# SmallVCM/SmallVCM

Hardware: AMD Instinct MI355X
Metric: Mpaths/sec (light+camera), VCM scene 1 at 2048^2 (higher is better)
Workload: dtype f32; 1 GPU; scene 1 -a vcm 2048x2048 maxPathLength 10 minPathLength 0 radiusFactor 0.003 radiusAlpha 0.75 seed 1234, iterations 5..408 timed; parallelism=1 renderer(s) (iteration-parallel, smallvcm.cxx:61-108) on one GPU, 1 in flight

## Files before the change

### smallvcm_amd/csrc/vcm_api.hip

```cpp
#include <hip/hip_runtime.h>
#include <stdio.h>
#include <stdlib.h>
#include <string.h>
#include <string>
#include <new>
#include <mutex>
#include <vector>
#include <condition_variable>
#include <atomic>

#include "vcm_kernels.h"
#include "vcm_kat.h"
#include "scene_host.h"
#include "scene_kind.h"
#include "vcm_denoise.h"
#include "vcm_variance.h"
#include "vcm_robust.h"
#include "vcm_parts.h"

using namespace vcm;

static thread_local std::string g_err;
static thread_local bool g_hipFailed;
static int fail(const char *what, const char *detail)
// ... 78 lines not shown
#endif
struct vcm_ctx : Scratch {
    SceneHost *scene;
    bool useVM, useVC, lightTraceOnly, ppm;
    int renderer;
    float baseRadius, radiusAlpha;
    int seed, device, rank, world;
    int resX, resY, N, p0, nLocal;
    int iterations;

    hipStream_t stream;
    bool ownStream;
    hipStream_t side;
    hipEvent_t evFork, evBbox, evGrid;
    bool gridInFlight;
    hipStream_t splat;
    hipEvent_t evSplatFork, evSplatDone;
    hipEvent_t evSortFork, evSorted;
    hipEvent_t evZero;
    bool prezeroed, sortInFlight;
    bool splatInFlight;
    bool resolveInFlight;
    hipEvent_t evMergeDone, evSplatWork, evResolved;
    hipEvent_t evPreMerge;
    bool mergeInFlight;
    bool deviceReady;
    ArenaPool *pool;
    Arena *arena; bool holdsArena;

    DScene *dScene;
    char *dSceneBlob;
    float *dFb;
    unsigned char *dRngLight, *dRngCam;
    GridHeader *dHdr;
    unsigned long long *dStats;
    unsigned long long *dStatsRing;
    unsigned long long *dStamps;
    float radiusRing[VCM_STAMP_RING];
    double stampKHz;

    bool importedRecords;
    bool importedSorted;
    bool sortedExchange;
    SortedSlabs sortedIn;
    SpaceSlabs space; bool spaceSet, mergeImported;
    float presetMin[3];
    int *dSpaceMatrix, *dSpaceScanned, *dSpaceTotals, *dSpaceHist;
    int *dWhereDest, *dWherePos; size_t whereCap;
    F4 *fQ, *fRes; int *fKey, *fArrival, *fSorted, *fCount; size_t fCap;
    bool gridBuilt, cameraTraced, merged, splatsPending, recordsValid, countedInCamera, scatteredInDI, bboxPreset;
    bool bboxFromLight;
    bool bboxFinal;
    bool strictOrder;
    int mergeKind;
    int lastMergeKernel;
    SceneKind kind;
    bool envMap;
    bool lens;
    bool filter;
    bool pick;
    bool lights;
    bool intPhong;
    F4 *dGuide, *dAlbedo;
    F4 *dDnA, *dDnB, *dDenoised;
    bool featuresValid, denoisedValid;
    bool trackVariance;
    F4 *dVarPrev, *dVarMom;
    int robustBuckets, robustAlloc;
    F4 *dRobPrev, *dRobBuckets, *dRobOut;
    bool trackParts;
    float *dParts;
    F4 *dPartOut;
    int fbIterations;
    IterParams P;
    bool inIteration;
    hipEvent_t ev[EV_COUNT];
    bool evValid;
    unsigned long long *pend[2][4]; int nPend[2];
    vcm_stats lastStats;
};

template <unsigned Wrap, class F> static void launch_kind(const vcm_ctx *c, F &&f) { with_scene_kind<Wrap>(c->kind, SceneWrappers{ c->lens || c->filter, c->pick, c->lights }, f); }

typedef void (*MergeKernel)(const DScene *, IterParams, GridStore, VertexStore, const int *, const int *, unsigned long long *, int, StampArgs);
static MergeKernel merge_kernel(int mergeKind, bool intPhong)
{
    if (mergeKind == VCM_MERGE_PAIRS) return intPhong ? k_merge_pairs<true> : k_merge_pairs<false>;
    return intPhong ? k_merge_walk<true> : k_merge_walk<false>;
}

static int use_device(vcm_ctx *c) { HIPCHK(hipSetDevice(c->device)); return 0; }

static thread_local size_t g_allocBytes;
template <typename T> static int dalloc(T **p, size_t n)
{
    void *v = NULL;
    HIPCHK(hipMalloc(&v, (n ? n : 1) * sizeof(T)));
    g_allocBytes += (n ? n : 1) * sizeof(T);
    *p = (T *)v;
    return 0;
}
#define DFREE(p) do { if (p) { (void)hipFree(p); p = NULL; } } while (0)

static std::mutex g_arenaRegistryMutex;
static ArenaPool *g_pools[64];

// ... 463 lines not shown
    vcm_ctx *c = new (std::nothrow) vcm_ctx();
    if (!c) { delete h; fail("vcm_create", "out of host memory"); return NULL; }
    memset((void *)c, 0, sizeof(*c));
    c->scene = h;
    c->envMap = h->envW > 0;
    c->lens = h->lensRadius > 0.f;
    c->filter = h->filterKind != VCM_FILTER_BOX;
    c->pick = h->pickMode != VCM_LIGHT_PICK_UNIFORM;
    c->lights = c->pick && scene_host_has_new_lights(*h);
    scene_host_build_accel(*h, scene_host_force_bvh());
    switch (algorithm) {
    case VCM_ALGO_LIGHT_TRACE: c->lightTraceOnly = true; break;
    case VCM_ALGO_PPM: c->ppm = true; c->useVM = true; break;
    case VCM_ALGO_BPM: c->useVM = true; break;
    case VCM_ALGO_BPT: c->useVC = true; break;
    case VCM_ALGO_VCM: c->useVC = true; c->useVM = true; break;
    case VCM_ALGO_PATH_TRACE: c->renderer = 1; break;
    case VCM_ALGO_EYE_LIGHT: c->renderer = 2; break;
    default: delete h; delete c; fail("vcm_create", "unknown algorithm"); return NULL;
    }
    if (c->ppm) {
        for (const vcm_material &m : h->materials) {
            const bool hasNonSpecular = (vmax3(ld3(m.diffuse)) > 0) || (vmax3(ld3(m.phong)) > 0);
            const bool hasSpecular = (vmax3(ld3(m.mirror)) > 0) || (m.ior > 0);
            if (hasNonSpecular && hasSpecular) {
                fprintf(stderr, "smallvcm_amd: scene mixes specular and non-specular BSDFs in one material, "
                                "switching from PPM to BPM (vertexcm.hxx:262-275)\n");
                c->ppm = false;
                break;
            }
        }
    }
    c->baseRadius = radiusFactor * h->sceneRadius;
    c->radiusAlpha = radiusAlpha;
    c->seed = seed;
    c->device = device; c->rank = rank; c->world = worldSize;
    c->resX = (int)h->camera.resolution[0];
    c->resY = (int)h->camera.resolution[1];
    c->N = c->resX * c->resY;
    if (c->N <= 0) { delete h; delete c; fail("vcm_create", "empty resolution"); return NULL; }
    c->p0 = (int)((long long)c->N * rank / worldSize);
    c->nLocal = (int)((long long)c->N * (rank + 1) / worldSize) - c->p0;
    c->ownStream = true;
    if (worldSize == 1) {
        c->pool = pool_get(device);
        if (!c->pool) { delete h; delete c; fail("vcm_create", "device index out of range"); return NULL; }
        std::lock_guard<std::mutex> g(c->pool->m);
        c->pool->users++;
    } else {
        c->arena = arena_new(device, NULL);
    }
    const char *so = getenv("SMALLVCM_AMD_STRICT_ORDER");
    c->strictOrder = (so && so[0] == '1');
    { const char *e = getenv("SMALLVCM_AMD_SORTED_EXCHANGE");
      c->sortedExchange = worldSize > 1 && worldSize <= VCM_SORTED_MAX_SHARDS && c->useVM && !(e && e[0] == '0'); }
    { const char *e = getenv("SMALLVCM_AMD_MERGE");
      c->mergeKind = (e && !strcmp(e, "walk")) ? VCM_MERGE_WALK : (e && !strcmp(e, "pairs")) ? VCM_MERGE_PAIRS : VCM_MERGE_DEFAULT; }
    c->lastMergeKernel = 0;
    return c;
}

vcm_ctx *vcm_create_sharded(const vcm_scene_desc *scene, int algorithm, float radiusFactor, float radiusAlpha,
                            int seed, int device, int rank, int worldSize)
{
    if (!scene) { fail("vcm_create", "scene is NULL"); return NULL; }
    SceneHost *h = new (std::nothrow) SceneHost();
    std::string err;
    if (!h || !scene_host_from_desc(*scene, *h, err)) { delete h; fail("vcm_create", err.c_str()); return NULL; }
    return create_from_host(h, algorithm, radiusFactor, radiusAlpha, seed, device, rank, worldSize);
}

vcm_ctx *vcm_create_sharded2(const vcm_scene_desc2 *scene, int algorithm, float radiusFactor, float radiusAlpha,
                             int seed, int device, int rank, int worldSize)
{
    if (!scene) { fail("vcm_create2", "scene is NULL"); return NULL; }
    SceneHost *h = new (std::nothrow) SceneHost();
    std::string err;
    if (!h || !scene_host_from_desc2(*scene, *h, err)) { delete h; fail("vcm_create2", err.c_str()); return NULL; }
    return create_from_host(h, algorithm, radiusFactor, radiusAlpha, seed, device, rank, worldSize);
}

vcm_ctx *vcm_create_sharded3(const vcm_scene_desc3 *scene, int algorithm, float radiusFactor, float radiusAlpha,
                             int seed, int device, int rank, int worldSize)
{
    if (!scene) { fail("vcm_create3", "scene is NULL"); return NULL; }
    SceneHost *h = new (std::nothrow) SceneHost();
    std::string err;
    if (!h || !scene_host_from_desc3(*scene, *h, err)) { delete h; fail("vcm_create3", err.c_str()); return NULL; }
    return create_from_host(h, algorithm, radiusFactor, radiusAlpha, seed, device, rank, worldSize);
}

vcm_ctx *vcm_create_sharded4(const vcm_scene_desc4 *scene, int algorithm, float radiusFactor, float radiusAlpha,
                             int seed, int device, int rank, int worldSize)
{
    if (!scene) { fail("vcm_create4", "scene is NULL"); return NULL; }
    SceneHost *h = new (std::nothrow) SceneHost();
    std::string err;
    if (!h || !scene_host_from_desc4(*scene, *h, err)) { delete h; fail("vcm_create4", err.c_str()); return NULL; }
    return create_from_host(h, algorithm, radiusFactor, radiusAlpha, seed, device, rank, worldSize);
}

vcm_ctx *vcm_create_sharded5(const vcm_scene_desc5 *scene, int algorithm, float radiusFactor, float radiusAlpha,
                             int seed, int device, int rank, int worldSize)
{
    if (!scene) { fail("vcm_create5", "scene is NULL"); return NULL; }
    SceneHost *h = new (std::nothrow) SceneHost();
// ... 320 lines not shown
        hipLaunchKernelGGL(k_splat_apply, dim3(aux_blocks(c->nLocal)), dim3(256), 0, q, c->N, (const int *)pixStart,
                           (const F4 *)list, c->dFb, arrival, pixCount, splatLong);
        hipLaunchKernelGGL(k_splat_apply_long, dim3(1024), dim3(256), 0, q, (const int *)pixStart, (const F4 *)list,
                           c->dSplat, c->dFb, (const int *)arrival, (const int *)pixCount);
        HIPCHK(hipGetLastError());
        if (c->trackParts) {
            float *plane = c->dParts + (size_t)VCM_PART_LIGHT_TRACE * (size_t)c->N * 3;
            HIPCHK(hipMemsetAsync(pixCount, 0, sizeof(int), q));
            hipLaunchKernelGGL(k_splat_apply, dim3(aux_blocks(c->nLocal)), dim3(256), 0, q, c->N, (const int *)pixStart,
                               (const F4 *)list, plane, arrival, pixCount, splatLong);
            hipLaunchKernelGGL(k_splat_apply_long, dim3(1024), dim3(256), 0, q, (const int *)pixStart, (const F4 *)list,
                               c->dSplat, plane, (const int *)arrival, (const int *)pixCount);
            HIPCHK(hipGetLastError());
        }
        if (overlap) {
            HIPCHK(hipEventRecord(c->evSplatDone, q));
            c->splatInFlight = true;
        }
    }
    return 0;
}

static int vcm_trace_light_impl(vcm_ctx *c)
{
    if (!c || !c->inIteration) return fail("vcm_trace_light", "no iteration in progress");
    if (use_device(c)) return -1;
    if (c->renderer) {
        if (mark(c, EV_LIGHT_K0)) return -1;
        if (mark(c, EV_LIGHT_K1)) return -1;
        HIPCHK(hipMemsetAsync(c->dLocalTotal, 0, sizeof(int), c->stream));
        if (mark(c, EV_LIGHT)) return -1;
        hipLaunchKernelGGL(k_set_counts, dim3(1), dim3(1), 0, c->stream, c->dHdr, c->dLocalTotal, 1, 0, take_stamps(c, c->stream));
        HIPCHK(hipGetLastError());
        return 0;
    }
    int blocks, chunk;
    trace_launch_shape(c->nLocal, &blocks, &chunk, true);
    if (c->world == 1 && !c->strictOrder) {
        HIPCHK(hipEventRecord(c->evFork, c->stream));
        HIPCHK(hipStreamWaitEvent(c->side, c->evFork, 0));
        if (zero_ranges(c->side, c->useVM ? c->dQueryCount : NULL, c->useVM ? ((size_t)c->P.nBuckets + 1) * sizeof(int) : 0,
                        (c->useVM && !grid_sort_is_radix(c)) ? c->dCellCount : NULL, c->useVM ? ((size_t)c->P.nCells + 1) * sizeof(int) : 0,
                        (c->useVC || c->lightTraceOnly) ? c->dPixCount : NULL, ((size_t)c->N + 1) * sizeof(int))) return -1;
        HIPCHK(hipEventRecord(c->evZero, c->side));
        c->prezeroed = true;
    }
    if (mark(c, EV_LIGHT_K0)) return -1;
    const bool wf = !c->strictOrder;
    if (!wf && join_splats(c)) return -1;
    if (wf)
        launch_kind<kWrapPick>(c, [&](auto tag) {
            using S = typename decltype(tag)::type;
            hipLaunchKernelGGL((k_light_trace<1, S>), dim3(blocks), dim3(VCM_TRACE_BLOCK), 0, c->stream, c->dScene, c->P, c->store,
                               c->dFb, c->dRngLight, c->dStats, chunk, take_stamps(c, c->stream), c->vs.count + 16, c->dHdr);
        });
    else
        launch_kind<kWrapLens | kWrapPick>(c, [&](auto tag) {
            using S = typename decltype(tag)::type;
            hipLaunchKernelGGL((k_light_trace<0, S>), dim3(blocks), dim3(VCM_TRACE_BLOCK), 0, c->stream, c->dScene, c->P, c->store,
                               c->dFb, c->dRngLight, c->dStats, chunk, take_stamps(c, c->stream), c->vs.count + 16, c->dHdr);
        });
    HIPCHK(hipGetLastError());
    c->bboxFromLight = c->world == 1;
    if (mark(c, EV_LIGHT_K1)) return -1;
    if (launch_scan<unsigned char>(c, c->store.count, c->nLocal, c->dPathStart, c->dLocalTotal, 0)) return -1;
    if (c->mergeInFlight) { HIPCHK(hipStreamWaitEvent(c->stream, c->evMergeDone, 0)); c->mergeInFlight = false; }
    bool countsSet = false;
    if (c->useVM || wf) {
        c->recordsValid = c->useVM && c->world > 1 && !c->sortedExchange;
        const bool fold = c->world == 1;
        hipLaunchKernelGGL(k_compact_records, dim3(aux_blocks(c->nLocal)), dim3(256), 0, c->stream, (const DScene *)c->dScene, c->P, c->store, c->dPathStart,
                           c->dRecordsLocal, c->dSlotOfVertex, c->recordsValid ? 1 : 0, fold ? c->dHdr : (GridHeader *)NULL,
                           (const int *)c->dLocalTotal, (fold && c->bboxFromLight) ? 1 : 0);
        HIPCHK(hipGetLastError());
        countsSet = fold;
        if (fold && c->bboxFromLight) c->bboxFinal = true;
    }
    if (wf && (c->useVC || c->lightTraceOnly)) {
        c->splatsPending = true;
        if (c->world == 1 && flush_light_splats(c)) return -1;
    }
    if (mark(c, EV_LIGHT)) return -1;
    if (!countsSet) {
        hipLaunchKernelGGL(k_set_counts, dim3(1), dim3(1), 0, c->stream, c->dHdr, c->dLocalTotal, 1, 0, take_stamps(c, c->stream));
        HIPCHK(hipGetLastError());
    }
    return 0;
}

static int ensure_records(vcm_ctx *c)
{
    if (c->recordsValid || !c->useVM) return 0;
    hipLaunchKernelGGL(k_compact_records, dim3(aux_blocks(c->nLocal)), dim3(256), 0, c->stream, (const DScene *)c->dScene, c->P, c->store, c->dPathStart,
                       c->dRecordsLocal, c->dSlotOfVertex, 1, (GridHeader *)NULL, (const int *)c->dLocalTotal, 0);
    HIPCHK(hipGetLastError());
    c->recordsValid = true;
    return 0;
}

int vcm_light_records(vcm_ctx *c, void **devPtr, long long *count)
{
    if (scratch_readable(c, "vcm_light_records")) return -1;
    if (use_device(c)) return -1;
    int n = 0;
    if (devPtr && ensure_records(c)) return -1;
    HIPCHK(hipMemcpyAsync(&n, c->dLocalTotal, sizeof(int), hipMemcpyDeviceToHost, c->stream));
    HIPCHK(hipStreamSynchronize(c->stream));
    if (devPtr) *devPtr = c->dRecordsLocal;
    if (count) *count = n;
    return 0;
}

static int vcm_local_light_bbox_impl(vcm_ctx *c, float *min3, float *max3, long long *count)
// ... 282 lines not shown
    return 0;
}

static GridStore grid_of(vcm_ctx *c)
{
    GridStore grid;
    grid.cellStart = c->dCellStart; grid.gx = c->dGx; grid.gy = c->dGy; grid.gz = c->dGz; grid.gb = c->dGb; grid.g1 = c->dG1; grid.g2 = c->dG2; grid.g3 = c->dG3;
    grid.hdr = c->dHdr;
    return grid;
}

static int vcm_trace_camera_impl(vcm_ctx *c)
{
    if (!c || !c->inIteration) return fail("vcm_trace_camera", "no iteration in progress");
    if (use_device(c)) return -1;
    if (flush_light_splats(c)) return -1;
    c->cameraTraced = true;
    if (c->lightTraceOnly) return 0;
    int blocks, chunk;
    trace_launch_shape(c->nLocal, &blocks, &chunk);
    if (c->resolveInFlight) HIPCHK(hipStreamWaitEvent(c->stream, c->evResolved, 0));
    if (mark(c, EV_CAMERA_K0)) return -1;
    if (c->renderer) {
        if (c->renderer == 1)
            launch_kind<kWrapLens | kWrapPick>(c, [&](auto tag) {
                using S = typename decltype(tag)::type;
                hipLaunchKernelGGL((k_path_trace<S>), dim3(blocks), dim3(VCM_TRACE_BLOCK), 0, c->stream, c->dScene, c->P, c->dCamOut,
                                   c->dRngCam, c->dStats, chunk, take_stamps(c, c->stream), c->vs.count + 8);
            });
        else
            launch_kind<kWrapLens>(c, [&](auto tag) {
                using S = typename decltype(tag)::type;
                hipLaunchKernelGGL((k_eye_light<S>), dim3(2048), dim3(256), 0, c->stream, c->dScene, c->P, c->dCamOut, c->dRngCam,
                                   c->dStats, take_stamps(c, c->stream));
            });
        HIPCHK(hipGetLastError());
        if (mark(c, EV_CAMERA_K1)) return -1;
        if (mark(c, EV_CONNECT_K1)) return -1;
        return 0;
    }
    if (c->P.wavefront) {
        c->countedInCamera = c->useVM && (c->gridBuilt || c->bboxPreset);
        c->vs.sortHdr = c->countedInCamera ? c->dHdr : NULL;
        c->vs.sortKey = c->countedInCamera ? c->dQueryKey : NULL;
        c->vs.sortArrival = c->countedInCamera ? c->dQueryArrival : NULL;
        c->vs.bucketCount = c->countedInCamera ? c->dQueryCount : NULL;
        if (c->countedInCamera) {
            if (c->prezeroed) HIPCHK(hipStreamWaitEvent(c->stream, c->evZero, 0));
            else if (zero_ranges(c->stream, c->dQueryCount, ((size_t)c->P.nBuckets + 1) * sizeof(int))) return -1;
        }
        launch_kind<kWrapLens | kWrapPick>(c, [&](auto tag) {
            using S = typename decltype(tag)::type;
            hipLaunchKernelGGL((k_camera_trace<1, S>), dim3(blocks), dim3(VCM_TRACE_BLOCK), 0, c->stream, c->dScene, c->P,
                               c->store, grid_of(c), c->vs, c->dCamOut, c->dCamMask, c->dRngCam, c->dStats, chunk, take_stamps(c, c->stream));
        });
        if (mark(c, EV_CAMERA_K1)) return -1;
        if (c->useVC) {
            c->scatteredInDI = c->countedInCamera && c->P.minLen <= 2;
            const bool inlineSort = c->scatteredInDI && (c->nLocal <= (1 << 20) || grid_sort_is_radix(c));
            if (c->countedInCamera && c->world == 1 && !inlineSort) {
                HIPCHK(hipEventRecord(c->evSortFork, c->stream));
                HIPCHK(hipStreamWaitEvent(c->side, c->evSortFork, 0));
                const StampArgs none = { { NULL, NULL, NULL, NULL } };
                if (launch_scan_on<int>(c, 3, c->side, c->dQueryCount, c->P.nBuckets, c->dQueryStart, NULL, 1, none)) return -1;
                hipLaunchKernelGGL(k_query_scatter, dim3(aux_blocks(c->nLocal)), dim3(256), 0, c->side, c->vs, (const int *)c->dQueryKey,
                                   (const int *)c->dQueryArrival, (const int *)c->dQueryStart, c->dSortedVertex);
                HIPCHK(hipEventRecord(c->evSorted, c->side));
                c->sortInFlight = true;
                c->scatteredInDI = false;
            }
            if (c->scatteredInDI && launch_scan<int>(c, c->dQueryCount, c->P.nBuckets, c->dQueryStart, NULL, 1)) return -1;
            {
                HIPCHK(hipEventRecord(c->evSplatFork, c->stream));
                HIPCHK(hipStreamWaitEvent(c->splat, c->evSplatFork, 0));
                launch_kind<kWrapNone>(c, [&](auto tag) {
                    using S = typename decltype(tag)::type;
                    hipLaunchKernelGGL((k_connect_vc<S>), dim3(task_blocks(c->nLocal)), dim3(VCM_TASK_BLOCK), 0, c->splat, c->dScene, c->P, c->vs,
                                       c->store, c->dStats);
                });
                HIPCHK(hipEventRecord(c->evSplatDone, c->splat));
                c->splatInFlight = true;
            }
            launch_kind<kWrapPick>(c, [&](auto tag) {
                using S = typename decltype(tag)::type;
                hipLaunchKernelGGL((k_connect_di<S>), dim3(task_blocks(c->nLocal)), dim3(VCM_TASK_BLOCK), 0, c->stream, c->dScene, c->P, c->vs,
                                   c->dStats, c->scatteredInDI ? (const int *)c->dQueryStart : (const int *)NULL,
                                   c->scatteredInDI ? c->dSortedVertex : (int *)NULL, take_stamps(c, c->stream));
            });
        }
        if (mark(c, EV_CONNECT_K1)) return -1;
    } else {
        if (c->useVM && !c->gridBuilt) return fail("vcm_trace_camera", "strict mode merges inside the camera pass: call vcm_build_grid first");
        launch_kind<kWrapLens | kWrapPick>(c, [&](auto tag) {
            using S = typename decltype(tag)::type;
            hipLaunchKernelGGL((k_camera_trace<0, S>), dim3(blocks), dim3(VCM_TRACE_BLOCK), 0, c->stream, c->dScene, c->P,
                               c->store, grid_of(c), c->vs, c->dCamOut, c->dCamMask, c->dRngCam, c->dStats, chunk, take_stamps(c, c->stream));
        });
        if (mark(c, EV_CAMERA_K1)) return -1;
        if (mark(c, EV_CONNECT_K1)) return -1;
    }
    HIPCHK(hipGetLastError());
    if (c->world > 1 && flush_stamps(c, c->stream)) return -1;
    return 0;
}

#define VCM_SPACE_BLOCKS 512
static int space_scratch(vcm_ctx *c)
{
    if (c->dSpaceMatrix) return 0;
    HIPCHK(hipMalloc((void **)&c->dSpaceMatrix, sizeof(int) * VCM_SPACE_MAX_SLABS * VCM_SPACE_BLOCKS));
    HIPCHK(hipMalloc((void **)&c->dSpaceScanned, sizeof(int) * (VCM_SPACE_MAX_SLABS * VCM_SPACE_BLOCKS + 1)));
    HIPCHK(hipMalloc((void **)&c->dSpaceTotals, sizeof(int) * VCM_SPACE_MAX_SLABS));
    HIPCHK(hipMalloc((void **)&c->dSpaceHist, sizeof(int) * 256));
    return 0;
}
static int space_ready(vcm_ctx *c, const char *who)
{
    if (!c || !c->inIteration) return fail(who, "no iteration in progress");
    if (c->world <= 1) return fail(who, "the context is not sharded");
    if (!c->useVM || !c->P.wavefront) return fail(who, "needs a merging algorithm in wavefront mode");
    if (use_device(c)) return -1;
    return space_scratch(c);
}
static int vcm_space_histogram_impl(vcm_ctx *c, int axis, float *lo, float *binWidth, int *hist256)
{
    if (space_ready(c, "vcm_space_histogram")) return -1;
    if (axis < 0 || axis > 2 || !lo || !binWidth || !hist256) return fail("vcm_space_histogram", "bad argument");
    if (ensure_records(c)) return -1;
    const float R = c->scene->sceneRadius, L = c->scene->sceneCenter[axis] - R, w = 2.f * R / 256.f;
    HIPCHK(hipMemsetAsync(c->dSpaceHist, 0, sizeof(int) * 256, c->stream));
    hipLaunchKernelGGL(k_space_hist, dim3(VCM_SPACE_BLOCKS), dim3(256), 0, c->stream, (const float *)c->dRecordsLocal, (const int *)c->dLocalTotal, axis, L, 1.f / w, c->dSpaceHist);
    HIPCHK(hipGetLastError());
    HIPCHK(hipMemcpyAsync(hist256, c->dSpaceHist, sizeof(int) * 256, hipMemcpyDeviceToHost, c->stream));
    HIPCHK(hipStreamSynchronize(c->stream));
    *lo = L; *binWidth = w;
    return 0;
}
static int vcm_space_set_slabs_impl(vcm_ctx *c, int axis, const float *splits, int nSlabs)
{
    if (space_ready(c, "vcm_space_set_slabs")) return -1;
    if (!c->bboxPreset) return fail("vcm_space_set_slabs", "call vcm_set_grid_bbox first: slabs are ranges of cells");
    if (axis < 0 || axis > 2 || !splits || nSlabs != c->world || nSlabs > VCM_SPACE_MAX_SLABS) return fail("vcm_space_set_slabs", "one slab per shard, at most 64");
    SpaceSlabs &sl = c->space;
    sl.S = nSlabs; sl.axis = axis;
    sl.X[0] = -(1 << 30); sl.X[nSlabs] = 1 << 30;
    for (int s2 = 1; s2 < nSlabs; s2++) {
        const float f = floorf(c->P.invCellSize * (splits[s2] - c->presetMin[axis]));
        int x = f < -1e9f ? -(1 << 30) : (f > 1e9f ? (1 << 30) : (int)f);
        if (x < sl.X[s2 - 1]) x = sl.X[s2 - 1];
// ... 1240 lines not shown
```

### smallvcm_amd/csrc/vcm_kernels.h

```cpp
#ifndef SMALLVCM_AMD_VCM_KERNELS_H
#define SMALLVCM_AMD_VCM_KERNELS_H

#include <hip/hip_runtime.h>
#include "vcm_core.h"

namespace vcm {

enum { STAT_LIGHT_RAYS = 0, STAT_CAMERA_RAYS, STAT_SHADOW_RAYS, STAT_MERGE_QUERIES, STAT_MERGE_CANDIDATES,
       STAT_MERGE_ACCEPTED, STAT_CONNECTIONS, STAT_LIGHT_SPLATS, STAT_STORED, STAT_COUNT };

#define VCM_TRACE_BLOCK 256
#define VCM_WAVE 64

struct StampArgs { unsigned long long *p[4]; };
__device__ __forceinline__ void stamp_entry(const StampArgs &s)
{
    if (blockIdx.x == 0 && threadIdx.x == 0 && s.p[0]) {
        const unsigned long long t = wall_clock64();
#pragma unroll
        for (int k = 0; k < 4; k++) if (s.p[k]) *s.p[k] = t;
    }
}

__device__ __forceinline__ unsigned lane_id() { return __builtin_amdgcn_mbcnt_hi(~0u, __builtin_amdgcn_mbcnt_lo(~0u, 0u)); }

__device__ __forceinline__ uint32_t wave_sum_u32(uint32_t v)
{
#pragma unroll
    for (int o = 32; o > 0; o >>= 1) v += __shfl_xor(v, o, 64);
    return v;
}

__device__ __forceinline__ void flush_stats(const LaneStats &ls, unsigned long long *g)
{
    const uint32_t v[STAT_COUNT] = { ls.lightRays, ls.cameraRays, ls.shadowRays, ls.mergeQueries, ls.mergeCandidates,
                                     ls.mergeAccepted, ls.connections, ls.lightSplats, ls.stored };
#pragma unroll
    for (int i = 0; i < STAT_COUNT; i++) {
        unsigned long long lo = wave_sum_u32(v[i] & 0xffffu);
        unsigned long long hi = wave_sum_u32(v[i] >> 16);
        const unsigned long long s = lo + (hi << 16);
        if (lane_id() == 0 && s) atomicAdd(&g[i], s);
    }
}

__device__ __forceinline__ uint32_t float_order_key(float f)
{
    const uint32_t u = f2u(f);
    return (u & 0x80000000u) ? ~u : (u | 0x80000000u);
}
__device__ __forceinline__ float float_from_order_key(uint32_t k)
{
    return u2f((k & 0x80000000u) ? (k & 0x7fffffffu) : ~k);
}

struct WaveWork { int next, end, dynBase; bool exhausted; };
__device__ __forceinline__ void wave_work_init(WaveWork &w, int chunk, int total)
{
    const int wave = (int)((blockIdx.x * blockDim.x + threadIdx.x) / VCM_WAVE), nWaves = (int)(gridDim.x * blockDim.x / VCM_WAVE);
    w.next = min(total, wave * chunk); w.end = min(total, w.next + chunk);
    w.dynBase = nWaves * chunk;
    w.exhausted = w.dynBase >= total;
}
__device__ __forceinline__ int wave_work_take(WaveWork &w, int *counter, int chunk, int total, unsigned long long need, unsigned lane)
{
    const int want = __popcll(need);
    const int rank = __popcll(need & ((1ull << lane) - 1ull));
    const int rem = max(w.end - w.next, 0);
    int idx = (rank < rem) ? w.next + rank : -1;
    if (want > rem && !w.exhausted) {
        int base = 0;
        if (lane == 0) base = atomicAdd(counter, chunk);
        base = w.dynBase + __builtin_amdgcn_readfirstlane(base);
        if (base >= total) w.exhausted = true;
        const int nend = min(total, base + chunk);
        if (rank >= rem) { const int i2 = base + (rank - rem); idx = (i2 < nend) ? i2 : -1; }
        w.next = base + (want - rem); w.end = nend;
    } else w.next += want;
    return idx;
}

#if defined(VCM_K1_WAVES)
#define VCM_K1_ATTR __attribute__((amdgpu_waves_per_eu(VCM_K1_WAVES, VCM_K1_WAVES)))
#else
#define VCM_K1_ATTR
#endif
template <int MODE, class SC>
__global__ void __launch_bounds__(VCM_TRACE_BLOCK) VCM_K1_ATTR
k_light_trace(const DScene *__restrict__ scp, IterParams P, LightStore store, float *fb,
              unsigned char *rngCount, unsigned long long *gstats, int chunk, StampArgs st, int *work, GridHeader *hdr)
{
    stamp_entry(st);
    const SC &sc = *static_cast<const SC *>(scp);
    stage_scene_tables(sc);
    stage_pick_tables(sc);
    const unsigned lane = lane_id();
    WaveWork ww; wave_work_init(ww, chunk, P.nLocal);
    LaneStats ls; lane_stats_zero(ls);
    LaneBox box; lane_box_init(box);
    LightPath path;
    bool alive = false;
    RC_DECL;
    for (;;) {
        const unsigned long long need = __builtin_amdgcn_ballot_w64(!alive);
        if (need) {
            const int idx = wave_work_take(ww, work, chunk, P.nLocal, need, lane);
            if (!alive && idx >= 0) { light_path_begin(sc, P, path, idx); alive = true; }
        }
        RC_MARK(19);
        if (!wave_any(alive)) { if (ww.exhausted) break; else continue; }
        if (alive) {
            alive = light_path_step<MODE>(sc, P, path, store, fb, ls, box);
            RC_RESET;
            if (!alive) {
                store.count[path.lp] = (unsigned char)path.nStored;
                store.lenMask[path.lp] = path.lenMask;
                rngCount[path.lp] = (unsigned char)path.rng.k;
            }
        }
        RC_MARK(21);
    }
    {
        uint32_t key[6];
#pragma unroll
        for (int c = 0; c < 3; c++) { key[c] = ~float_order_key(box.mn[c]); key[3 + c] = float_order_key(box.mx[c]); }
        __shared__ uint32_t sbox[VCM_TRACE_BLOCK / VCM_WAVE][6];
#pragma unroll
        for (int c = 0; c < 6; c++) {
#pragma unroll
            for (int o = 32; o > 0; o >>= 1) key[c] = max(key[c], (uint32_t)__shfl_xor((int)key[c], o, 64));
            if (lane == 0) sbox[threadIdx.x / VCM_WAVE][c] = key[c];
        }
        __syncthreads();
        if (threadIdx.x < 6) {
            uint32_t v = sbox[0][threadIdx.x];
            for (int w = 1; w < VCM_TRACE_BLOCK / VCM_WAVE; w++) v = max(v, sbox[w][threadIdx.x]);
            if (threadIdx.x < 3) atomicMax(&hdr->bboxMinU[threadIdx.x], v); else atomicMax(&hdr->bboxMaxU[threadIdx.x - 3], v);
        }
    }
    flush_stats(ls, gstats);
}

#if defined(VCM_K3_WAVES)
#define VCM_K3_ATTR __attribute__((amdgpu_waves_per_eu(VCM_K3_WAVES, VCM_K3_WAVES)))
#else
#define VCM_K3_ATTR
#endif
template <int MODE, class SC>
__global__ void __launch_bounds__(VCM_TRACE_BLOCK) VCM_K3_ATTR
k_camera_trace(const DScene *__restrict__ scp, IterParams P, LightStore store, GridStore grid, VertexStore vs,
               F4 *camOut, uint32_t *camMask, unsigned char *rngCount, unsigned long long *gstats, int chunk, StampArgs st)
{
    stamp_entry(st);
    const SC &sc = *static_cast<const SC *>(scp);
    stage_scene_tables(sc);
    stage_pick_tables(sc);
    const unsigned lane = lane_id();
    WaveWork ww; wave_work_init(ww, chunk, P.nLocal);
    int *work = vs.count + 8;
    LaneStats ls; lane_stats_zero(ls);
    __shared__ uint32_t accQ[MODE == 1 ? 1 : (VCM_MERGE_Q + 1) * VCM_TRACE_BLOCK];
    MergeScratch ms; ms.q = accQ + (MODE == 1 ? 0 : threadIdx.x); ms.stride = VCM_TRACE_BLOCK; ms.cap = VCM_MERGE_Q;
    __shared__ int wqState[(VCM_TRACE_BLOCK / VCM_WAVE) * 6];
    int *myState = wqState + (threadIdx.x / VCM_WAVE) * 6;
    if (lane < 6) myState[lane] = 0;
    CameraWaveQueues wqs;
    wqs.v.p = (WaveQueueWords)myState; wqs.di.p = (WaveQueueWords)(myState + 2); wqs.vc.p = (WaveQueueWords)(myState + 4);
    wqs.pendingVertex = -1; wqs.pendingArrival = 0;
    QueryKey qk = { 0.f, 0.f, 0.f, 0.f, 0.f, 0.f, 1u, 1u, 0, 0, 0 };
    if (MODE == 1 && vs.sortKey && P.useVM) qk = query_key_load(P, vs.sortHdr);
    CameraPath path;
    bool alive = false;
    RC_DECL;
    for (;;) {
        const unsigned long long need = __builtin_amdgcn_ballot_w64(!alive);
        if (need) {
            const int idx = wave_work_take(ww, work, chunk, P.nLocal, need, lane);
            if (!alive && idx >= 0) { camera_path_begin(sc, P, path, idx, MODE == 1 ? store.lenMask : (const uint32_t *)0); alive = true; }
        }
        RC_MARK(20);
        if (!wave_any(alive)) { if (ww.exhausted) break; else continue; }
        if (alive) {
            alive = camera_path_step<MODE>(sc, P, path, store, grid, ls, ms, vs, wqs, qk);
            RC_RESET;
            if (!alive) {
                const int target = camera_path_target(P, path);
                camOut[path.lp] = mk4(path.color.x, path.color.y, path.color.z, u2f((uint32_t)target));
                if (MODE == 1) camMask[path.lp] = path.queryMask;
                rngCount[path.lp] = (unsigned char)path.rng.k;
            }
        }
        RC_MARK(22);
    }
    if (MODE == 1 && wqs.pendingVertex >= 0) vs.sortArrival[wqs.pendingVertex] = wqs.pendingArrival;
    if (MODE == 1) {
        const int vb = wq_load(wqs.v.p), vl = wq_load(wqs.v.p + 1), db = wq_load(wqs.di.p), dl = wq_load(wqs.di.p + 1), cb = wq_load(wqs.vc.p), cl = wq_load(wqs.vc.p + 1);
        for (int i = (int)lane; i < vl; i += VCM_WAVE) {
            vq(vs, 0, vb + i) = mk4(0.f, 0.f, 0.f, u2f(0xffffffffu));
            if (vs.sortKey) vs.sortKey[vb + i] = -1;
        }
        for (int i = (int)lane; i < dl; i += VCM_WAVE) vs.diTask[db + i] = -1;
        for (int i = (int)lane; i < cl; i += VCM_WAVE) vs.vcTask[2 * (cb + i)] = -1;
    }
    flush_stats(ls, gstats);
}

template <class SC>
__global__ void __launch_bounds__(VCM_TRACE_BLOCK)
k_path_trace(const DScene *__restrict__ scp, IterParams P, F4 *camOut, unsigned char *rngCount,
             unsigned long long *gstats, int chunk, StampArgs st, int *work)
{
    stamp_entry(st);
    const SC &sc = *static_cast<const SC *>(scp);
    stage_scene_tables(sc);
    stage_pick_tables(sc);
    const unsigned lane = lane_id();
    WaveWork ww; wave_work_init(ww, chunk, P.nLocal);
    LaneStats ls; lane_stats_zero(ls);
    PtPath path;
    bool alive = false;
    for (;;) {
        const unsigned long long need = __builtin_amdgcn_ballot_w64(!alive);
        if (need) {
            const int idx = wave_work_take(ww, work, chunk, P.nLocal, need, lane);
            if (!alive && idx >= 0) { pt_path_begin(sc, P, path, idx); alive = true; }
        }
        if (!wave_any(alive)) { if (ww.exhausted) break; else continue; }
        if (alive) {
            alive = pt_path_step(sc, P, path, ls);
            if (!alive) {
                camOut[path.lp] = mk4(path.color.x, path.color.y, path.color.z, u2f((uint32_t)raster_target(P, path.sx, path.sy)));
                rngCount[path.lp] = (unsigned char)path.rng.k;
            }
        }
// ... 1451 lines not shown
```

Measured before the change: 1265 Mpaths/s.

## Compact sparse tail waves by migrating live paths through LDS mailboxes

Once a wave has no more work to take and its live-lane count drops to a threshold or below, it packs its surviving light or camera paths into a per-wave LDS mailbox and retires. Sibling waves with dead lanes claim those paths and continue tracing them, so fewer waves sit mostly empty at the end of the persistent loop. The light kernel's bbox reduction also drops its __syncthreads in favour of LDS atomics, with the last-finishing wave publishing the result. The cost is larger LDS use, pack/unpack traffic, RNG re-init on unpack, and subtle atomic ordering that could hurt occupancy or introduce races.

```diff
diff --git a/smallvcm_amd/csrc/vcm_api.hip b/smallvcm_amd/csrc/vcm_api.hip
--- a/smallvcm_amd/csrc/vcm_api.hip
+++ b/smallvcm_amd/csrc/vcm_api.hip
@@ -154,6 +154,7 @@
     bool bboxFromLight;
     bool bboxFinal;
     bool strictOrder;
+    int tailLanes;
     int mergeKind;
     int lastMergeKernel;
     SceneKind kind;
@@ -723,6 +724,8 @@
     }
     const char *so = getenv("SMALLVCM_AMD_STRICT_ORDER");
     c->strictOrder = (so && so[0] == '1');
+    { const char *e = getenv("SMALLVCM_AMD_TAIL_COMPACT");
+      c->tailLanes = !e ? VCM_TAIL_DEFAULT : (atoi(e) < 0 ? 0 : (atoi(e) > VCM_TAIL_BOX ? VCM_TAIL_BOX : atoi(e))); }
     { const char *e = getenv("SMALLVCM_AMD_SORTED_EXCHANGE");
       c->sortedExchange = worldSize > 1 && worldSize <= VCM_SORTED_MAX_SHARDS && c->useVM && !(e && e[0] == '0'); }
     { const char *e = getenv("SMALLVCM_AMD_MERGE");
@@ -1149,13 +1152,13 @@
         launch_kind<kWrapPick>(c, [&](auto tag) {
             using S = typename decltype(tag)::type;
             hipLaunchKernelGGL((k_light_trace<1, S>), dim3(blocks), dim3(VCM_TRACE_BLOCK), 0, c->stream, c->dScene, c->P, c->store,
-                               c->dFb, c->dRngLight, c->dStats, chunk, take_stamps(c, c->stream), c->vs.count + 16, c->dHdr);
+                               c->dFb, c->dRngLight, c->dStats, chunk, take_stamps(c, c->stream), c->vs.count + 16, c->dHdr, c->tailLanes);
         });
     else
         launch_kind<kWrapLens | kWrapPick>(c, [&](auto tag) {
             using S = typename decltype(tag)::type;
             hipLaunchKernelGGL((k_light_trace<0, S>), dim3(blocks), dim3(VCM_TRACE_BLOCK), 0, c->stream, c->dScene, c->P, c->store,
-                               c->dFb, c->dRngLight, c->dStats, chunk, take_stamps(c, c->stream), c->vs.count + 16, c->dHdr);
+                               c->dFb, c->dRngLight, c->dStats, chunk, take_stamps(c, c->stream), c->vs.count + 16, c->dHdr, c->tailLanes);
         });
     HIPCHK(hipGetLastError());
     c->bboxFromLight = c->world == 1;
@@ -1544,7 +1547,7 @@
         launch_kind<kWrapLens | kWrapPick>(c, [&](auto tag) {
             using S = typename decltype(tag)::type;
             hipLaunchKernelGGL((k_camera_trace<1, S>), dim3(blocks), dim3(VCM_TRACE_BLOCK), 0, c->stream, c->dScene, c->P,
-                               c->store, grid_of(c), c->vs, c->dCamOut, c->dCamMask, c->dRngCam, c->dStats, chunk, take_stamps(c, c->stream));
+                               c->store, grid_of(c), c->vs, c->dCamOut, c->dCamMask, c->dRngCam, c->dStats, chunk, take_stamps(c, c->stream), c->tailLanes);
         });
         if (mark(c, EV_CAMERA_K1)) return -1;
         if (c->useVC) {
@@ -1586,7 +1589,7 @@
         launch_kind<kWrapLens | kWrapPick>(c, [&](auto tag) {
             using S = typename decltype(tag)::type;
             hipLaunchKernelGGL((k_camera_trace<0, S>), dim3(blocks), dim3(VCM_TRACE_BLOCK), 0, c->stream, c->dScene, c->P,
-                               c->store, grid_of(c), c->vs, c->dCamOut, c->dCamMask, c->dRngCam, c->dStats, chunk, take_stamps(c, c->stream));
+                               c->store, grid_of(c), c->vs, c->dCamOut, c->dCamMask, c->dRngCam, c->dStats, chunk, take_stamps(c, c->stream), c->tailLanes);
         });
         if (mark(c, EV_CAMERA_K1)) return -1;
         if (mark(c, EV_CONNECT_K1)) return -1;
diff --git a/smallvcm_amd/csrc/vcm_kernels.h b/smallvcm_amd/csrc/vcm_kernels.h
--- a/smallvcm_amd/csrc/vcm_kernels.h
+++ b/smallvcm_amd/csrc/vcm_kernels.h
@@ -3,6 +3,7 @@
 
 #include <hip/hip_runtime.h>
 #include "vcm_core.h"
+#include "vcm_tail.h"
 
 namespace vcm {
 
@@ -80,6 +81,120 @@
     return idx;
 }
 
+struct TailWord {
+    WaveQueueWords p;
+    __device__ __forceinline__ int load_relaxed() const { return __hip_atomic_load(p, __ATOMIC_RELAXED, __HIP_MEMORY_SCOPE_WORKGROUP); }
+    __device__ __forceinline__ int fetch_sub_acq_rel(int k) const { return __hip_atomic_fetch_add(p, -k, __ATOMIC_ACQ_REL, __HIP_MEMORY_SCOPE_WORKGROUP); }
+    __device__ __forceinline__ void store_release(int v) const { __hip_atomic_store(p, v, __ATOMIC_RELEASE, __HIP_MEMORY_SCOPE_WORKGROUP); }
+};
+template <class PATH> struct TailWords;
+template <> struct TailWords<CameraPath> {
+    enum { N = 23 };
+    static __device__ __forceinline__ void pack(const CameraPath &p, uint32_t *w)
+    {
+        const SubPathState &s = p.st;
+        w[0] = f2u(s.origin.x); w[1] = f2u(s.origin.y); w[2] = f2u(s.origin.z);
+        w[3] = f2u(s.direction.x); w[4] = f2u(s.direction.y); w[5] = f2u(s.direction.z);
+        w[6] = f2u(s.throughput.x); w[7] = f2u(s.throughput.y); w[8] = f2u(s.throughput.z);
+        w[9] = s.pathLength; w[10] = s.specularPath; w[11] = f2u(s.dVCM); w[12] = f2u(s.dVC); w[13] = f2u(s.dVM);
+        w[14] = p.rng.k; w[15] = f2u(p.color.x); w[16] = f2u(p.color.y); w[17] = f2u(p.color.z); w[18] = (uint32_t)p.lp;
+        w[19] = f2u(p.sx); w[20] = f2u(p.sy); w[21] = p.queryMask; w[22] = p.lightLenMask;
+    }
+    static __device__ __forceinline__ void unpack(const uint32_t *w, const IterParams &P, CameraPath &p)
+    {
+        SubPathState &s = p.st;
+        s.origin = mk3(u2f(w[0]), u2f(w[1]), u2f(w[2])); s.direction = mk3(u2f(w[3]), u2f(w[4]), u2f(w[5]));
+        s.throughput = mk3(u2f(w[6]), u2f(w[7]), u2f(w[8]));
+        s.pathLength = w[9]; s.specularPath = w[10]; s.isFiniteLight = 0u; s.dVCM = u2f(w[11]); s.dVC = u2f(w[12]); s.dVM = u2f(w[13]);
+        p.color = mk3(u2f(w[15]), u2f(w[16]), u2f(w[17])); p.lp = (int)w[18];
+        p.sx = u2f(w[19]); p.sy = u2f(w[20]); p.queryMask = w[21]; p.lightLenMask = w[22];
+        rng_init(p.rng, P.seed, P.localIter, (uint32_t)(P.p0 + p.lp), 1u); p.rng.k = w[14];
+    }
+};
+template <> struct TailWords<LightPath> {
+    enum { N = 18 };
+    static __device__ __forceinline__ void pack(const LightPath &p, uint32_t *w)
+    {
+        const SubPathState &s = p.st;
+        w[0] = f2u(s.origin.x); w[1] = f2u(s.origin.y); w[2] = f2u(s.origin.z);
+        w[3] = f2u(s.direction.x); w[4] = f2u(s.direction.y); w[5] = f2u(s.direction.z);
+        w[6] = f2u(s.throughput.x); w[7] = f2u(s.throughput.y); w[8] = f2u(s.throughput.z);
+        w[9] = s.pathLength; w[10] = s.isFiniteLight; w[11] = f2u(s.dVCM); w[12] = f2u(s.dVC); w[13] = f2u(s.dVM);
+        w[14] = p.rng.k; w[15] = (uint32_t)p.lp; w[16] = (uint32_t)p.nStored; w[17] = p.lenMask;
+    }
+    static __device__ __forceinline__ void unpack(const uint32_t *w, const IterParams &P, LightPath &p)
+    {
+        SubPathState &s = p.st;
+        s.origin = mk3(u2f(w[0]), u2f(w[1]), u2f(w[2])); s.direction = mk3(u2f(w[3]), u2f(w[4]), u2f(w[5]));
+        s.throughput = mk3(u2f(w[6]), u2f(w[7]), u2f(w[8]));
+        s.pathLength = w[9]; s.isFiniteLight = w[10]; s.specularPath = 0u; s.dVCM = u2f(w[11]); s.dVC = u2f(w[12]); s.dVM = u2f(w[13]);
+        p.lp = (int)w[15]; p.nStored = (int)w[16]; p.lenMask = w[17];
+        rng_init(p.rng, P.seed, P.localIter, (uint32_t)(P.p0 + p.lp), 0u); p.rng.k = w[14];
+    }
+};
+static_assert(sizeof(CameraPath) == 28 * 4 && sizeof(LightPath) == 23 * 4 && sizeof(SubPathState) == 15 * 4 && sizeof(PathRng) == 5 * 4,
+              "a member was added to a path state: decide in TailWords whether it travels");
+template <class PATH, int SLOTS>
+struct TailLds {
+    enum { WORDS = TailWords<PATH>::N };
+    int running, done, cnt[VCM_TAIL_WAVES];
+    uint32_t box[VCM_TAIL_WAVES][WORDS][SLOTS];
+};
+template <class PATH, int SLOTS>
+__device__ __forceinline__ void tail_lds_init(TailLds<PATH, SLOTS> &tl)
+{
+    if (threadIdx.x == 0) { tl.running = (int)(blockDim.x / VCM_WAVE); tl.done = 0; }
+    if (threadIdx.x < VCM_TAIL_WAVES) tl.cnt[threadIdx.x] = 0;
+}
+template <class PATH, int SLOTS>
+__device__ __forceinline__ bool wave_tail_step(TailLds<PATH, SLOTS> &tl, const IterParams &P, int threshold, unsigned lane, PATH &path, bool &alive, bool &last)
+{
+    enum { WORDS = TailLds<PATH, SLOTS>::WORDS };
+    const int self = __builtin_amdgcn_readfirstlane((int)(threadIdx.x / VCM_WAVE));
+    for (;;) {
+        unsigned long long dead = __builtin_amdgcn_ballot_w64(!alive);
+        for (int b = 0; b < VCM_TAIL_WAVES && dead; b++) {
+            if (b == self && !last) continue;
+            int first = 0, got = 0;
+            if (lane == 0) { TailWord w = { (WaveQueueWords)&tl.cnt[b] }; got = tail_claim(w, (int)__popcll(dead), first); }
+            got = __builtin_amdgcn_readfirstlane(got); first = __builtin_amdgcn_readfirstlane(first);
+            if (!got) continue;
+            __builtin_amdgcn_fence(__ATOMIC_ACQUIRE, "workgroup");
+            const int rank = (int)lanes_below_mask_popc(dead);
+            if (!alive && rank < got) {
+                uint32_t w[WORDS];
+#pragma unroll
+                for (int i = 0; i < WORDS; i++) w[i] = tl.box[b][i][first + rank];
+                TailWords<PATH>::unpack(w, P, path);
+                alive = true;
+            }
+            dead = __builtin_amdgcn_ballot_w64(!alive);
+        }
+        const unsigned long long live = __builtin_amdgcn_ballot_w64(alive);
+        const int n = (int)__popcll(live);
+        if (last) return n == 0;
+        if (n > threshold) return false;
+        if (alive) {
+            uint32_t w[WORDS];
+            TailWords<PATH>::pack(path, w);
+            const int slot = (int)lanes_below_mask_popc(live);
+#pragma unroll
+            for (int i = 0; i < WORDS; i++) tl.box[self][i][slot] = w[i];
+        }
+        alive = false;
+        __builtin_amdgcn_fence(__ATOMIC_RELEASE, "workgroup");
+        int isLast = 0;
+        if (lane == 0) {
+            TailWord c = { (WaveQueueWords)&tl.cnt[self] }; tail_publish(c, n);
+            TailWord r = { (WaveQueueWords)&tl.running }; isLast = tail_leave(r) ? 1 : 0;
+        }
+        if (!__builtin_amdgcn_readfirstlane(isLast)) return true;
+        last = true;
+    }
+}
+template <class SC> struct TailSlots { enum { value = SC::kBvh ? 4 : VCM_TAIL_BOX }; };
+template <int MODE> struct TailInK3 { enum { value = MODE == 1 }; };
+
 #if defined(VCM_K1_WAVES)
 #define VCM_K1_ATTR __attribute__((amdgpu_waves_per_eu(VCM_K1_WAVES, VCM_K1_WAVES)))
 #else
@@ -88,10 +203,16 @@
 template <int MODE, class SC>
 __global__ void __launch_bounds__(VCM_TRACE_BLOCK) VCM_K1_ATTR
 k_light_trace(const DScene *__restrict__ scp, IterParams P, LightStore store, float *fb,
-              unsigned char *rngCount, unsigned long long *gstats, int chunk, StampArgs st, int *work, GridHeader *hdr)
+              unsigned char *rngCount, unsigned long long *gstats, int chunk, StampArgs st, int *work, GridHeader *hdr,
+              int tailT )
 {
     stamp_entry(st);
     const SC &sc = *static_cast<const SC *>(scp);
+    __shared__ TailLds<LightPath, TailSlots<SC>::value> tl;
+    __shared__ uint32_t sbox[6];
+    tail_lds_init(tl);
+    if (threadIdx.x < 6) sbox[threadIdx.x] = 0u;
+    tailT = min(tailT, (int)TailSlots<SC>::value);
     stage_scene_tables(sc);
     stage_pick_tables(sc);
     const unsigned lane = lane_id();
@@ -99,7 +220,7 @@
     LaneStats ls; lane_stats_zero(ls);
     LaneBox box; lane_box_init(box);
     LightPath path;
-    bool alive = false;
+    bool alive = false, tailLast = false;
     RC_DECL;
     for (;;) {
         const unsigned long long need = __builtin_amdgcn_ballot_w64(!alive);
@@ -108,7 +229,9 @@
             if (!alive && idx >= 0) { light_path_begin(sc, P, path, idx); alive = true; }
         }
         RC_MARK(19);
-        if (!wave_any(alive)) { if (ww.exhausted) break; else continue; }
+        if (tailT > 0 && ww.exhausted && ww.next >= ww.end) {
+            if (wave_tail_step(tl, P, tailT, lane, path, alive, tailLast)) break;
+        } else if (!wave_any(alive)) { if (ww.exhausted) break; else continue; }
         if (alive) {
             alive = light_path_step<MODE>(sc, P, path, store, fb, ls, box);
             RC_RESET;
@@ -124,18 +247,20 @@
         uint32_t key[6];
 #pragma unroll
         for (int c = 0; c < 3; c++) { key[c] = ~float_order_key(box.mn[c]); key[3 + c] = float_order_key(box.mx[c]); }
-        __shared__ uint32_t sbox[VCM_TRACE_BLOCK / VCM_WAVE][6];
 #pragma unroll
         for (int c = 0; c < 6; c++) {
 #pragma unroll
             for (int o = 32; o > 0; o >>= 1) key[c] = max(key[c], (uint32_t)__shfl_xor((int)key[c], o, 64));
-            if (lane == 0) sbox[threadIdx.x / VCM_WAVE][c] = key[c];
-        }
-        __syncthreads();
-        if (threadIdx.x < 6) {
-            uint32_t v = sbox[0][threadIdx.x];
-            for (int w = 1; w < VCM_TRACE_BLOCK / VCM_WAVE; w++) v = max(v, sbox[w][threadIdx.x]);
-            if (threadIdx.x < 3) atomicMax(&hdr->bboxMinU[threadIdx.x], v); else atomicMax(&hdr->bboxMaxU[threadIdx.x - 3], v);
+            if (lane == 0) __hip_atomic_fetch_max(&sbox[c], key[c], __ATOMIC_RELAXED, __HIP_MEMORY_SCOPE_WORKGROUP);
+        }
+        int before = 0;
+        if (lane == 0) before = __hip_atomic_fetch_add((WaveQueueWords)&tl.done, 1, __ATOMIC_ACQ_REL, __HIP_MEMORY_SCOPE_WORKGROUP);
+        if (__builtin_amdgcn_readfirstlane(before) == (int)(blockDim.x / VCM_WAVE) - 1) {
+            __builtin_amdgcn_fence(__ATOMIC_ACQUIRE, "workgroup");
+            if (lane < 6) {
+                const uint32_t v = __hip_atomic_load(&sbox[lane], __ATOMIC_RELAXED, __HIP_MEMORY_SCOPE_WORKGROUP);
+                if (lane < 3) atomicMax(&hdr->bboxMinU[lane], v); else atomicMax(&hdr->bboxMaxU[lane - 3], v);
+            }
         }
     }
     flush_stats(ls, gstats);
@@ -149,10 +274,14 @@
 template <int MODE, class SC>
 __global__ void __launch_bounds__(VCM_TRACE_BLOCK) VCM_K3_ATTR
 k_camera_trace(const DScene *__restrict__ scp, IterParams P, LightStore store, GridStore grid, VertexStore vs,
-               F4 *camOut, uint32_t *camMask, unsigned char *rngCount, unsigned long long *gstats, int chunk, StampArgs st)
+               F4 *camOut, uint32_t *camMask, unsigned char *rngCount, unsigned long long *gstats, int chunk, StampArgs st,
+               int tailT )
 {
     stamp_entry(st);
     const SC &sc = *static_cast<const SC *>(scp);
+    __shared__ TailLds<CameraPath, TailInK3<MODE>::value ? TailSlots<SC>::value : 1> tl;
+    tail_lds_init(tl);
+    tailT = TailInK3<MODE>::value ? min(tailT, (int)TailSlots<SC>::value) : 0;
     stage_scene_tables(sc);
     stage_pick_tables(sc);
     const unsigned lane = lane_id();
@@ -170,7 +299,7 @@
     QueryKey qk = { 0.f, 0.f, 0.f, 0.f, 0.f, 0.f, 1u, 1u, 0, 0, 0 };
     if (MODE == 1 && vs.sortKey && P.useVM) qk = query_key_load(P, vs.sortHdr);
     CameraPath path;
-    bool alive = false;
+    bool alive = false, tailLast = false;
     RC_DECL;
     for (;;) {
         const unsigned long long need = __builtin_amdgcn_ballot_w64(!alive);
@@ -179,7 +308,9 @@
             if (!alive && idx >= 0) { camera_path_begin(sc, P, path, idx, MODE == 1 ? store.lenMask : (const uint32_t *)0); alive = true; }
         }
         RC_MARK(20);
-        if (!wave_any(alive)) { if (ww.exhausted) break; else continue; }
+        if (TailInK3<MODE>::value && tailT > 0 && ww.exhausted && ww.next >= ww.end) {
+            if (wave_tail_step(tl, P, tailT, lane, path, alive, tailLast)) break;
+        } else if (!wave_any(alive)) { if (ww.exhausted) break; else continue; }
         if (alive) {
             alive = camera_path_step<MODE>(sc, P, path, store, grid, ls, ms, vs, wqs, qk);
             RC_RESET;
diff --git a/smallvcm_amd/csrc/vcm_tail.h b/smallvcm_amd/csrc/vcm_tail.h
--- /dev/null
+++ b/smallvcm_amd/csrc/vcm_tail.h
@@ -0,0 +1,41 @@
+#ifndef SMALLVCM_AMD_VCM_TAIL_H
+#define SMALLVCM_AMD_VCM_TAIL_H
+
+#define VCM_TAIL_WAVES 4
+#define VCM_TAIL_BOX 32
+#define VCM_TAIL_DEFAULT 16
+
+#if defined(__HIPCC__)
+#define VCM_TAIL_FN __host__ __device__ __forceinline__
+#else
+#define VCM_TAIL_FN inline
+#endif
+
+namespace vcm {
+
+template <class Word>
+VCM_TAIL_FN int tail_claim(Word &cnt, int k, int &first)
+{
+    first = 0;
+    if (k <= 0 || cnt.load_relaxed() <= 0) return 0;
+    const int old = cnt.fetch_sub_acq_rel(k);
+    if (old <= 0) return 0;
+    const int got = old < k ? old : k;
+    first = old - got;
+    return got;
+}
+
+template <class Word>
+VCM_TAIL_FN void tail_publish(Word &cnt, int n)
+{
+    if (n > 0) cnt.store_release(n);
+}
+
+template <class Word>
+VCM_TAIL_FN bool tail_leave(Word &running)
+{
+    return running.fetch_sub_acq_rel(1) == 1;
+}
+
+}
+#endif
```

New measurement: 1257 Mpaths/s. Within noise of the previous version (-0.6%).
